# shenwei356/wfa

Hardware: AMD Instinct MI355X
Metric: aligned pairs/sec (and Gcells/s) on 1e6 synthetic 1 kbp pairs @5% error (higher is better)
Workload: dtype u32; 1 GPU; 1000000 x 1000 bp pairs/GPU @5% error, global gap-affine 4/6/2, wf-adaptive 10/50/1, seed 3; config=c3, pairs_per_gpu=1000000, length=1000, parallelism=pair-sharded x1, ranks_seen_by_collective=1, backend=none (1 GPU), collective_forced=False, status_ok=1000000, setup_steps=0, gather=none (1 GPU), gather_bytes_per_rank_step=0, packed_pairs=1000000, retried_pairs=831

## Files before the change

### wfa_amd/csrc/wfa_blk.hpp

```cpp
#pragma once
#include "wfa_device.hpp"
#include "wfa_packed.hpp"
#include <type_traits>

namespace wfa {

#ifndef WFA_BLK_TILED
#define WFA_BLK_TILED 1
#endif

template <int G>
struct BlkOps;

template <>
struct BlkOps<16> {
    static WFA_DEV uint32_t dn1(uint32_t x, int) { return (uint32_t)__builtin_amdgcn_update_dpp(0, (int)x, 0x111, 0xf, 0xf, true); }
    static WFA_DEV uint32_t up1(uint32_t x, int) { return (uint32_t)__builtin_amdgcn_update_dpp(0, (int)x, 0x101, 0xf, 0xf, true); }
#ifndef WFA_BLK_SHIFT_LANES
#define WFA_BLK_SHIFT_LANES 1
#endif
    static constexpr int SHIFT_D = 4 * WFA_BLK_SHIFT_LANES;
    static WFA_DEV uint32_t shr(uint32_t x, int) { return (uint32_t)__builtin_amdgcn_update_dpp(0, (int)x, 0x110 + WFA_BLK_SHIFT_LANES, 0xf, 0xf, true); }
    static WFA_DEV uint32_t shl(uint32_t x, int) { return (uint32_t)__builtin_amdgcn_update_dpp(0, (int)x, 0x100 + WFA_BLK_SHIFT_LANES, 0xf, 0xf, true); }
};

// ... 1045 lines not shown
        for (int i = 0; i < 8; i++) atomicAdd(acc + 8 + i, evt[i]);
    }
#endif
    if constexpr (STREAM) {
        stream_backtrace(P);
    }
    if constexpr (G == 64 && PP == 1 && !LONG) {
        if (P.fuse_bt) {
            if constexpr (LDSA) {
                __builtin_amdgcn_fence(__ATOMIC_ACQ_REL, "workgroup");
                if (lds[P.lds_arena_off - 4] != ST_OK) __threadfence();
                backtrace_wave_one<true>(P, blockIdx.x, lds + P.lds_arena_off);
            } else {
                __threadfence();
            }
            if constexpr (LDSA) {
            } else
                for (uint32_t idx = blockIdx.x; idx < P.chunk_n; idx += gridDim.x) backtrace_wave_one(P, idx, lds);
            if (lane == 0 && gridDim.x == 1u) *P.queue_head = 0u, *P.redo_count = 0u, *P.ops_cursor = 0ull;
        }
    }
}

WFA_DEV uint32_t prepack_dword(uint32_t w, bool &bad) {
    const uint32_t x = (w >> 1) & 0x03030303u;
    bad |= __builtin_amdgcn_perm(0u, 0x47544341u, x) != w;
    const uint32_t y = x | (x >> 6);
    return (y & 0xFu) | ((y >> 12) & 0xF0u);
}
WFA_DEV void prepack_fetch(const uint8_t *blob, uint64_t off, uint32_t len, uint32_t jw, uint32_t (&d)[5], uint32_t &sh, uint32_t &nb) {
    const uint32_t nw = (len + 15u) >> 4;
    sh = 0u, nb = 0u;
#pragma unroll
    for (int i = 0; i < 5; i++) d[i] = 0u;
    if (jw >= nw) return;
    const uintptr_t a  = (uintptr_t)(blob + off) + 16ull * jw;
    const uint32_t *p  = (const uint32_t *)(a & ~(uintptr_t)3);
    sh = (uint32_t)(a & 3) * 8u;
    nb = (len - 16u * jw) < 16u ? (len - 16u * jw) : 16u;
    const uint32_t  nd = ((uint32_t)(a & 3) + nb + 3u) >> 2;
    if ((a & 15) == 0 && nb == 16u) {
        const uint4 v = *reinterpret_cast<const uint4 *>(a);
        d[0] = v.x, d[1] = v.y, d[2] = v.z, d[3] = v.w, d[4] = 0u;
    } else {
#pragma unroll
        for (int i = 0; i < 5; i++) d[i] = ((uint32_t)i < nd) ? p[i] : 0u;
    }
}
WFA_DEV uint32_t prepack_finish(const uint32_t (&d)[5], uint32_t sh, uint32_t nb, bool &bad) {
    if (nb == 0u) return 0u;
    uint32_t word = 0u;
#pragma unroll
    for (int i = 0; i < 4; i++) {
        uint32_t w = __funnelshift_r(d[i], d[i + 1], sh);
        if (nb < 16u) {
            const uint32_t mb = nb > 4u * i ? (nb - 4u * i < 4u ? nb - 4u * i : 4u) : 0u;
            const uint32_t km = mb >= 4u ? 0xFFFFFFFFu : ((1u << (8u * mb)) - 1u);
            w = (w & km) | (0x41414141u & ~km);
        }
        word |= prepack_dword(w, bad) << (8 * i);
    }
    return word;
}
WFA_DEV uint32_t prepack_word(const uint8_t *blob, uint64_t off, uint32_t len, uint32_t jw, bool &bad) {
    uint32_t d[5], sh, nb;
    prepack_fetch(blob, off, len, jw, d, sh, nb);
    return prepack_finish(d, sh, nb, bad);
}

constexpr int PREPACK_PAIRS = 4;
#ifndef WFA_NO_AUX_KERNELS
__global__ __launch_bounds__(256) void wfa_prepack_kernel(const KParams P, uint32_t *out, uint32_t SW, uint32_t PW, uint32_t ppw) {
    const uint32_t lane = threadIdx.x & 63u;
    const uint32_t wv   = blockIdx.x * 4u + (threadIdx.x >> 6);
    const uint32_t LP = 2u * SW <= 32u ? 32u : 64u, side = lane / LP, v0 = lane % LP, n_side = 64u / LP;
    struct Hd { uint32_t nq, mt; uint64_t qo, to; };
    const auto load_hd = [&](uint32_t k) -> Hd {
        const uint32_t wi = wv * ppw + k + side;
        Hd h = {0u, 0u, 0ull, 0ull};
        if (k < ppw && wi < P.chunk_n) {
            const uint32_t pr = P.work ? P.work[wi] : P.chunk_first + wi;
            h.nq = P.q_len[pr], h.mt = P.t_len[pr], h.qo = P.q_off[pr], h.to = P.t_off[pr];
        }
        return h;
    };
    Hd nxt = load_hd(0);
    for (uint32_t k = 0; k < ppw; k += n_side) {
        const uint32_t wi = wv * ppw + k + side;
        if (wv * ppw + k >= P.chunk_n) return;
        const bool     have = wi < P.chunk_n;
        const Hd       cur  = nxt;
        nxt                 = load_hd(k + n_side);
// ... 32 lines not shown
```

### wfa_amd/csrc/wfa_ctx.hpp

```cpp
#pragma once
#include "../../include/wfa_hip.h"
#include "wfa_common.hpp"

#include <algorithm>
#include <atomic>
#include <chrono>
#include <cmath>
#include <cstdio>
#include <cstdlib>
#include <cstring>
#include <deque>
#include <functional>
#include <malloc.h>
#include <mutex>
#include <new>
#include <numeric>
#include <string>
#include <thread>
#include <vector>
#include <fcntl.h>
#include <optional>
#include <sys/file.h>
#include <unistd.h>

// ... 111 lines not shown
    int64_t       opt_arena_poison         = 0;
    int64_t       opt_pilot                = 1;
    int64_t       opt_tail_overlap         = 1;
    int64_t       opt_overlap              = 0;
    int64_t       opt_fail_pass            = 0;
    int64_t       opt_prepack              = 0;
    int64_t       opt_narrow_long          = 0;
    DevBuf        score_out;
    DevBuf        wide_ckpt;
    DevBuf        mx_seq, mx_words;
    DevBuf        mx_out;
    uint2        *mx_pin       = nullptr;
    size_t        mx_pin_bytes = 0;
    hipEvent_t    mx_ev[4]     = {};
    int64_t       opt_matrix_tile_cells    = 0;
    int64_t       opt_wide                 = 1;
    int64_t       opt_wide_max_len         = 2047;
    int           opt_wide_waves           = 0;
    bool          opt_wide_exact           = false;
    int64_t       opt_wide_min_pairs       = 64;
    int64_t       opt_duo                  = 1;
    int64_t       opt_duo_min_pairs        = 200000;
    bool          opt_duo_pk               = true;
    int64_t       opt_duo_short            = 0;
    int64_t       opt_duo_short_min_pairs  = 50000;
    bool          ctrl_clean               = false;
    hipStream_t   ctrl_clean_stream        = nullptr;
    hipEvent_t    ctrl_clean_ev            = nullptr;
    bool          redo_was_empty           = false;
    int64_t       opt_compact_call_bases   = 50000000;
    int64_t       opt_lane                 = 1;
    int64_t       opt_lane_pack            = 1;
    int64_t       opt_lane_min_pairs       = 32768;
    int64_t       opt_long                 = 1;
    int64_t       opt_long_min_len         = 4000;
    int64_t       opt_long_window_words    = 240;
    int64_t       opt_long_first           = 0;
    int64_t       opt_long_wave_bt         = 1;
    int64_t       opt_census               = 0;
    int64_t       opt_learn                = 1;
    uint64_t      learn_key                = 0;
    int           learn_level              = 0;
    uint32_t      learn_calls              = 0;
    uint64_t      rows_key                 = 0;
    uint32_t      rows_scale               = 1;
    uint64_t      band_key                 = 0;
// ... 59 lines not shown
```

### wfa_amd/csrc/wfa_duo.hip

```cpp
#define WFA_NO_AUX_KERNELS 1
#include "wfa_duo.hpp"
#include "wfa_fwd.hpp"

namespace wfa {

namespace {
template <int DX, int DOE>
hipError_t go_duo(const KParams &P, uint32_t grid, size_t lds_bytes, hipStream_t st, bool census, bool pk) {
    if (pk && census)
        hipLaunchKernelGGL((wfa_duo_kernel<true, DX, DOE>), dim3(grid), dim3(64), lds_bytes, st, P);
    else if (pk)
        hipLaunchKernelGGL((wfa_duo_kernel<false, DX, DOE>), dim3(grid), dim3(64), lds_bytes, st, P);
    else if (census)
        hipLaunchKernelGGL((wfa_duo32_kernel<true, DX, DOE>), dim3(grid), dim3(64), lds_bytes, st, P);
    else
        hipLaunchKernelGGL((wfa_duo32_kernel<false, DX, DOE>), dim3(grid), dim3(64), lds_bytes, st, P);
    return hipGetLastError();
}
}

hipError_t wfa_launch_duo(int shape, const KParams &P, uint32_t grid, size_t lds_bytes, hipStream_t st, bool census, bool pk) {
    switch (shape) {
    case 0: return go_duo<2, 4>(P, grid, lds_bytes, st, census, pk);
    case 1: return go_duo<1, 3>(P, grid, lds_bytes, st, census, pk);
    case 2: return go_duo<1, 2>(P, grid, lds_bytes, st, census, pk);
    case 3: return go_duo<2, 3>(P, grid, lds_bytes, st, census, pk);
    case 4: return go_duo<2, 2>(P, grid, lds_bytes, st, census, pk);
    case 5: return go_duo<3, 3>(P, grid, lds_bytes, st, census, pk);
    }
    return hipErrorInvalidValue;
}

}
```

### wfa_amd/csrc/wfa_duo.hpp

```cpp
#pragma once
#include "wfa_blk.hpp"
#include "wfa_duo_cfg.hpp"
#include "wfa_pk16.hpp"

namespace wfa {

struct DuoRed {
#define WFA_DUO_3(opa, opb, opc)                                                                                    \
    unsigned long long sv;                                                                                          \
    asm volatile("s_nop 1\n\t" opa " %0, %0, %0 " WFA_DPP_CTL_XOR1 "\n\t" opb " %1, %1, %1 " WFA_DPP_CTL_XOR1 "\n\t" opc \
        " %2, %2, %2 " WFA_DPP_CTL_XOR1 "\n\t" opa " %0, %0, %0 " WFA_DPP_CTL_XOR2 "\n\t" opb " %1, %1, %1 "        \
        WFA_DPP_CTL_XOR2 "\n\t" opc " %2, %2, %2 " WFA_DPP_CTL_XOR2 "\n\t" opa " %0, %0, %0 " WFA_DPP_CTL_HMIR "\n\t" \
        opb " %1, %1, %1 " WFA_DPP_CTL_HMIR "\n\t" opc " %2, %2, %2 " WFA_DPP_CTL_HMIR "\n\t"                         \
        "s_and_saveexec_b64 %3, %4\n\t" opa " %0, %0, %0 " WFA_DPP_CTL_MIR "\n\t" opb " %1, %1, %1 " WFA_DPP_CTL_MIR    \
        "\n\t" opc " %2, %2, %2 " WFA_DPP_CTL_MIR "\n\ts_mov_b64 exec, %3"                                            \
        : "+v"(a), "+v"(b), "+v"(c), "=&s"(sv)                                                                      \
        : "s"(wm)                                                                                                   \
        : "scc");
#define WFA_DUO_2(opa, opb)                                                                                         \
    unsigned long long sv;                                                                                          \
    asm volatile("s_nop 1\n\t" opa " %0, %0, %0 " WFA_DPP_CTL_XOR1 "\n\t" opb " %1, %1, %1 " WFA_DPP_CTL_XOR1 "\n\ts_nop 0\n\t" \
        opa " %0, %0, %0 " WFA_DPP_CTL_XOR2 "\n\t" opb " %1, %1, %1 " WFA_DPP_CTL_XOR2 "\n\ts_nop 0\n\t" opa        \
        " %0, %0, %0 " WFA_DPP_CTL_HMIR "\n\t" opb " %1, %1, %1 " WFA_DPP_CTL_HMIR "\n\t"                            \
        "s_and_saveexec_b64 %2, %3\n\t" opa " %0, %0, %0 " WFA_DPP_CTL_MIR "\n\t" opb " %1, %1, %1 " WFA_DPP_CTL_MIR    \
// ... 5 lines not shown
    unsigned long long sv;                                                                                          \
    asm volatile("s_nop 1\n\t" opa " %0, %0, %0 " WFA_DPP_CTL_XOR1 "\n\ts_nop 1\n\t" opa " %0, %0, %0 " WFA_DPP_CTL_XOR2 \
        "\n\ts_nop 1\n\t" opa " %0, %0, %0 " WFA_DPP_CTL_HMIR "\n\t"                                                \
        "s_and_saveexec_b64 %1, %2\n\ts_nop 0\n\t" opa " %0, %0, %0 " WFA_DPP_CTL_MIR "\n\ts_mov_b64 exec, %1"       \
        : "+v"(a), "=&s"(sv)                                                                                        \
        : "s"(wm)                                                                                                   \
        : "scc");
    static WFA_DEV void min_max_min(int &a, int &b, int &c, unsigned long long wm) { WFA_DUO_3("v_min_i32_dpp", "v_max_i32_dpp", "v_min_i32_dpp") }
    static WFA_DEV void min_max(int &a, int &b, unsigned long long wm) { WFA_DUO_2("v_min_i32_dpp", "v_max_i32_dpp") }
    static WFA_DEV void max_add(int &a, int &b, unsigned long long wm) { WFA_DUO_2("v_max_i32_dpp", "v_add_u32_dpp") }
    static WFA_DEV int  max1(int a, unsigned long long wm) {
        WFA_DUO_1("v_max_i32_dpp")
        return a;
    }
    static WFA_DEV int or1(int a, unsigned long long wm) {
        WFA_DUO_1("v_or_b32_dpp")
        return a;
    }
#undef WFA_DUO_3
#undef WFA_DUO_2
#undef WFA_DUO_1
};

template <bool CENSUS, int DX, int DOE, bool PK>
__device__ __attribute__((always_inline)) inline void duo_run(const KParams &P) {
    constexpr int PP = 4;
    static_assert(DX >= 1 && DOE >= 1 && DX <= 4 && DOE <= 4, "ring depths of one to four score steps");
    constexpr int R  = DX > DOE ? DX : DOE;
    constexpr int RW = PK ? 2 : PP;
    extern __shared__ __attribute__((aligned(16))) uint32_t lds[];
    const int  lane = threadIdx.x, l7 = lane & 7, l15 = lane & 15;
    const bool hi_half = (lane & 8) != 0;

    const uint32_t  SW = P.lds_seq_words, PW = P.prepack_words;
    const uint32_t  FP = duo_fetch_pairs(PW), NBUF = duo_bufs(PW);
    uint32_t *const park0 = lds + NBUF * PW;
    const uint64_t  cap      = P.arena_words;
    const int       mdd      = (int)P.max_dist_diff;
    const int       minwf    = (int)P.min_wf_len;
    const bool      adaptive = P.adaptive != 0;
    const uint32_t  seed_si  = P.dx;
    uint32_t        pk_one   = 0x00010001u;
    if constexpr (PK) asm volatile("" : "+s"(pk_one));
    const int       rows_cap = (int)(cap / 32);

    int       st = 0;
    bool      wide = false;
    uint32_t  pidx = 0, si = 0, cells = 0, sbuf = 0;
    int       n = 0, m = 0, kb = 0;
    bool      slow = false, first_eq = false;
    int             j = l7, k0 = 0;
    uint32_t        mdn = 0u, mup = 0u;
    const uint32_t *lq = lds + 4, *lt = lds + 4;
    uint32_t       *rowp = nullptr;

    uint32_t M[R][RW], I[RW], D[RW];
    int      rlo[R], rhi[R];
    int      lim[PP], lmx[PP];
#pragma unroll
    for (int d = 0; d < R; d++) {
        rlo[d] = BK_BIG, rhi[d] = -BK_BIG;
#pragma unroll
        for (int p = 0; p < RW; p++) M[d][p] = 0u;
    }
#pragma unroll
    for (int p = 0; p < RW; p++) I[p] = D[p] = 0u;
#pragma unroll
    for (int p = 0; p < PP; p++) lim[p] = 0, lmx[p] = 0;

    uint32_t buf_free  = (1u << NBUF) - 1u;
    uint32_t park_used = 0u;
    constexpr uint32_t PF_TOK = 1u, PF_LD = 2u, PF_STAGED = 4u, PF_DRY = 8u;
    uint32_t pf = 0u;
    uint32_t pf_tok = 0u, pf_ld_idx = 0u, pf_idx = 0u, pf_buf = 0u;
    uint32_t st_mask = 0u;
    uint4    pf_w = make_uint4(0u, 0u, 0u, 0u);

#ifdef WFA_STAMPS
    unsigned long long stamp_acc[8] = {0, 0, 0, 0, 0, 0, 0, 0}, stamp_prev;
    unsigned long long evt[8] = {0, 0, 0, 0, 0, 0, 0, 0};
    asm volatile("s_memtime %0\n\ts_waitcnt lgkmcnt(0)" : "=s"(stamp_prev)::"memory");
#endif
    const auto pair_of = [&](uint32_t idx) { return P.work ? P.work[idx] : P.chunk_first + idx; };
    const auto dn1 = [&](uint32_t x) { return (uint32_t)__builtin_amdgcn_update_dpp(0, (int)x, 0x111, 0xf, 0xf, true) & mdn; };
    const auto up1 = [&](uint32_t x) { return (uint32_t)__builtin_amdgcn_update_dpp(0, (int)x, 0x101, 0xf, 0xf, true) & mup; };
    const auto other_half = [&](int x) { return __builtin_amdgcn_update_dpp(0, x, 0x128, 0xf, 0xf, true); };
    const auto set_derived = [&]() {
        j   = wide ? l15 : l7;
        mdn = j == 0 ? 0u : ~0u;
        mup = j == (wide ? 15 : 7) ? 0u : ~0u;
        k0  = kb + PP * j;
#pragma unroll
        for (int p = 0; p < PP; p++) lim[p] = imax2(1, imin2(n + k0 + p, m)), lmx[p] = imax2(n + k0 + p, m);
        lq   = lds + sbuf * PW + 4u;
        lt   = lq + SW;
        if constexpr (DUO_ARENA_FMT == 10u)
            rowp = P.arena + (uint64_t)pidx * cap + (((uint32_t)k0 & 56u) >> 3) * (uint32_t)(rows_cap * 4) + (((uint32_t)k0 >> 2) & 1u) * 16u;
        else if constexpr (DUO_ARENA_FMT == 9u)
            rowp = P.arena + (uint64_t)pidx * cap + (((uint32_t)k0 & 60u) >> 2) * (uint32_t)(rows_cap * 2) + si * 2u;
        else
            rowp = P.arena + (uint64_t)pidx * cap + (uint64_t)(si >> 3) * 256u + (si & 7u) * 2u;
    };
    const auto clear_rings = [&]() {
#pragma unroll
        for (int d = 0; d < R; d++) {
            rlo[d] = BK_BIG, rhi[d] = -BK_BIG;
#pragma unroll
            for (int p = 0; p < RW; p++) M[d][p] = 0u;
        }
#pragma unroll
        for (int p = 0; p < RW; p++) I[p] = D[p] = 0u;
    };
    const auto or_halves = [&](uint32_t v) {
        uint32_t r = 0u;
#pragma unroll
        for (int o = 0; o < 8; o++) r |= (uint32_t)__builtin_amdgcn_readlane((int)v, 8 * o);
        return r;
    };

    const auto refill = [&](auto ph_c) __attribute__((always_inline)) -> bool {
        constexpr int ph  = decltype(ph_c)::value;
        constexpr int NEW = (ph + R - 1) % R;
        pf        = (uint32_t)__builtin_amdgcn_readfirstlane((int)pf);
        park_used = (uint32_t)__builtin_amdgcn_readfirstlane((int)park_used);
        buf_free  = (uint32_t)__builtin_amdgcn_readfirstlane((int)buf_free);
        st_mask   = (uint32_t)__builtin_amdgcn_readfirstlane((int)st_mask);
        if ((pf & (PF_LD | PF_STAGED)) == PF_LD) {
            const uint32_t cnt = umin2(FP, P.chunk_n - pf_ld_idx);
            st_mask = 0u;
            {
                uint32_t f = buf_free;
                for (uint32_t c = 0; c < cnt; c++) st_mask |= f & (0u - f), f &= f - 1u;
            }
            buf_free &= ~st_mask;
            const uint32_t w0 = (uint32_t)lane * 4u, slot = w0 / PW;
            if (slot < cnt) {
                uint32_t f = st_mask;
                for (uint32_t c = 0; c < slot; c++) f &= f - 1u;
                const uint32_t b = (uint32_t)__builtin_ctz(f);
                *reinterpret_cast<uint4 *>(lds + b * PW + (w0 - slot * PW)) = pf_w;
            }
            pf_idx = pf_ld_idx, pf = (pf | PF_STAGED) & ~PF_LD;
        }
        if ((pf & (PF_TOK | PF_LD)) == PF_TOK) {
            pf_ld_idx = (uint32_t)__builtin_amdgcn_readfirstlane((int)pf_tok);
            const bool have = pf_ld_idx < P.chunk_n;
            if (have) {
                const uint32_t *const slot = P.prepack + (uint64_t)pf_ld_idx * PW;
                const uint32_t cnt = umin2(FP, P.chunk_n - pf_ld_idx);
                if ((uint32_t)lane * 4u < cnt * PW) pf_w = *reinterpret_cast<const uint4 *>(slot + lane * 4);
            }
            pf = (pf & ~PF_TOK) | (have ? PF_LD : PF_DRY);
        }
        if ((pf & (PF_TOK | PF_DRY)) == 0u) {
            if (lane == 0) pf_tok = atomicAdd(P.queue_head, FP);
            pf |= PF_TOK;
        }
        unsigned long long m_free;
        WFA_STAMP(0);
        for (;;) {
        const bool run   = st == 1;
        const int  Wc    = wide ? 64 : 32;
        const bool touch = run && rhi[NEW] >= rlo[NEW] && (rlo[NEW] <= kb || rhi[NEW] >= kb + Wc - 1);
        bool       narrowable = false;
        if constexpr (ph == 0) {
            int ulo = rlo[0], uhi = rhi[0];
#pragma unroll
            for (int d = 1; d < R; d++) ulo = imin2(ulo, rlo[d]), uhi = imax2(uhi, rhi[d]);
            narrowable    = run && wide && uhi - ulo + 1 <= DUO_NARROW_AT;
        }
        const unsigned long long m_ev = __ballot(touch || narrowable);
        m_free = __ballot(st == 0);
        if (__builtin_expect(!(m_ev != 0ull || (m_free != 0ull && (park_used != 0u || (pf & PF_STAGED) != 0u))), 1)) break;
        WFA_EVT(1, 1);
        {
// ... 189 lines not shown
                    }
                    buf_free |= 1u << pf_buf;
                    continue;
                }
                WFA_EVT(5, 1);
                if (mine) {
                    pidx = this_idx, sbuf = pf_buf;
                    n = (int)nq, m = (int)mt;
                    const int Ak = m - n;
                    si = 0, cells = 0, slow = false;
                    kb = -16 + PP * imax2(-3, imin2(3, Ak / (2 * PP)));
                    first_eq = ((hb[4] ^ hb[4 + SW]) & 3u) == 0u;
                    clear_rings();
                    st = 1, wide = false;
                }
                m_free &= ~(0xFFull << (8 * oct));
            }
            set_derived();
            __builtin_amdgcn_fence(__ATOMIC_RELEASE, "wavefront");
            __builtin_amdgcn_fence(__ATOMIC_ACQUIRE, "wavefront");
        }
        }
        WFA_STAMP(1);
        return m_free == ~0ull && park_used == 0u && (pf & (PF_DRY | PF_LD | PF_STAGED)) == PF_DRY;
    };

    const auto step = [&](auto ph_c) __attribute__((always_inline)) {
        constexpr int ph = decltype(ph_c)::value;
        const bool run = (st == 1);
        const unsigned long long wm = __ballot(wide);
        WFA_EVT(0, 1), WFA_EVT(6, __builtin_popcountll(__ballot(run)) / 8);

        uint32_t(&Mo)[RW] = M[(ph + R - DOE) % R];
        uint32_t(&Mx)[RW] = M[(ph + R - DX) % R];
        uint32_t(&Mn)[RW] = M[ph];

        uint32_t nM[PP], nI[RW], nD[RW], wd[RW], cc[PP];
        const uint32_t a_edge = dn1(Mo[RW - 1]), b_edge = dn1(I[RW - 1]);
        const uint32_t c_edge = up1(Mo[0]), d_edge = up1(D[0]);
        const bool     slow_any = __ballot(run && slow) != 0ull;
        const auto next_slow = [&](const uint32_t(&Mo4)[PP], const uint32_t(&I4)[PP], const uint32_t(&D4)[PP], const uint32_t(&Mx4)[PP],
                                   uint32_t ae, uint32_t be, uint32_t ce, uint32_t de, uint32_t(&nI4)[PP], uint32_t(&nD4)[PP],
                                   uint32_t(&wd4)[PP]) __attribute__((always_inline)) {
#pragma unroll
            for (int p = 0; p < PP; p++) {
                const int      k  = k0 + p;
                const uint32_t a0 = p ? Mo4[p - 1] : ae, b0 = p ? I4[p - 1] : be;
// ... 289 lines not shown
            if (refill(std::integral_constant<int, 2 % R>{})) break;
            step(std::integral_constant<int, 2 % R>{});
        }
        if constexpr (R > 3) {
            if (refill(std::integral_constant<int, 3 % R>{})) break;
            step(std::integral_constant<int, 3 % R>{});
        }
    }
#ifdef WFA_STAMPS
    if (lane == 0 && P.debug_info) {
        unsigned long long *acc = reinterpret_cast<unsigned long long *>(P.debug_info);
        for (int i = 0; i < 8; i++) atomicAdd(acc + i, stamp_acc[i]);
        for (int i = 0; i < 8; i++) atomicAdd(acc + 8 + i, evt[i]);
    }
#endif
}

#ifndef WFA_DUO_VGPRS
#define WFA_DUO_VGPRS 64
#endif
static_assert(16u * (256u - 4u) / 2u < 2048u, "wfa_duo_kernel's packed rings need offsets under 4 096");
template <bool CENSUS, int DX = 2, int DOE = 4>
__global__ __launch_bounds__(64, WFA_DUO_WAVES) __attribute__((amdgpu_num_vgpr(WFA_DUO_VGPRS))) void wfa_duo_kernel(const KParams P) {
    duo_run<CENSUS, DX, DOE, true>(P);
}
template <bool CENSUS, int DX = 2, int DOE = 4>
__global__ __launch_bounds__(64, WFA_DUO_WAVES) __attribute__((amdgpu_num_vgpr(WFA_DUO_VGPRS))) void wfa_duo32_kernel(const KParams P) {
    duo_run<CENSUS, DX, DOE, false>(P);
}

}
```

### wfa_amd/csrc/wfa_host.hip

```cpp
#include <map>
#include "wfa_ctx.hpp"
#include "wfa_generic.hpp"
#include "wfa_packed.hpp"
#include "wfa_reg.hpp"
#include "wfa_blk.hpp"
#include "wfa_duo_cfg.hpp"
#include "wfa_lane.hpp"
#include "wfa_team.hpp"
#include "wfa_teamc.hpp"
#include "wfa_fwd.hpp"
#include "wfa_long.hpp"
#include "wfa_wide.hpp"

using namespace wfa;
static_assert(TEAM_SOLO_MAX == 4096, "wfa_ctx.hpp: default of opt_team_solo_max");

namespace wfa {
hipError_t wfa_launch_fwd(int shape, int kind, uint32_t flags, const KParams &P, uint32_t grid, size_t lds_bytes, hipStream_t st) {
    switch (shape) {
    case 0: return wfa_launch_fwd_s24(kind, flags, P, grid, lds_bytes, st);
    case 1: return wfa_launch_fwd_s13(kind, flags, P, grid, lds_bytes, st);
    case 2: return wfa_launch_fwd_s12(kind, flags, P, grid, lds_bytes, st);
    case 3: return wfa_launch_fwd_s23(kind, flags, P, grid, lds_bytes, st);
    case 4: return wfa_launch_fwd_s22(kind, flags, P, grid, lds_bytes, st);
// ... 382 lines not shown
        ctx->opt_pair_lds = value, ctx->one_lds_skip = 0;
    else if (k == "long_wave_bt")
        ctx->opt_long_wave_bt = value;
    else if (k == "long_min_len")
        ctx->opt_long_min_len = value;
    else if (k == "long_window_words")
        ctx->opt_long_window_words = (value >= 64 && value <= 4096 && value % 4 == 0) ? value : 240;
    else if (k == "wide")
        ctx->opt_wide = value;
    else if (k == "wide_min_pairs")
        ctx->opt_wide_min_pairs = value;
    else if (k == "matrix_tile_cells")
        ctx->opt_matrix_tile_cells = value > 0 ? value : 0;
    else if (k == "wide_max_len")
        ctx->opt_wide_max_len = value;
    else if (k == "wide_exact")
        ctx->opt_wide_exact = value != 0;
    else if (k == "wide_waves")
        ctx->opt_wide_waves = (value == 1 || value == 4) ? (int)value : 0;
    else if (k == "duo")
        ctx->opt_duo = value;
    else if (k == "duo_pk")
        ctx->opt_duo_pk = value != 0;
    else if (k == "duo_min_pairs")
        ctx->opt_duo_min_pairs = value;
    else if (k == "compact_call_bases")
        ctx->opt_compact_call_bases = value;
    else if (k == "lane")
        ctx->opt_lane = value;
    else if (k == "lane_pack")
        ctx->opt_lane_pack = value;
    else if (k == "lane_min_pairs")
        ctx->opt_lane_min_pairs = value;
    else if (k == "duo_short")
        ctx->opt_duo_short = value;
    else if (k == "duo_short_min_pairs")
        ctx->opt_duo_short_min_pairs = value;
    else if (k == "blk_mid")
        ctx->opt_blk_mid = value;
    else if (k == "pair_fast")
        ctx->opt_pair_fast = value;
    else if (k == "arena_budget_pct")
        ctx->opt_arena_budget_pct = value;
    else if (k == "autopack")
        ctx->opt_autopack = value;
    else if (k == "learn")
// ... 267 lines not shown
        HIP_TRY(hipMemsetAsync(stampbuf.p, 0, 128, st));
        P.debug_info = static_cast<uint32_t *>(stampbuf.p);
#endif
        uint64_t rkey = 0;
        {
            uint32_t lb = 0;
            while ((2u << lb) <= max_len) lb++;
            rkey = 1ull | ((uint64_t)lb << 1) | ((uint64_t)P.adaptive << 9) | ((uint64_t)(P.x & 0xFFF) << 12) | ((uint64_t)(P.oe & 0xFFF) << 24) |
                   ((uint64_t)(P.e & 0xFFF) << 36) | ((uint64_t)(P.max_dist_diff & 0xFFFF) << 48);
        }
        uint64_t arena_mult = (ctx->rows_key == rkey && ctx->opt_packed_arena_bytes <= 0) ? ctx->rows_scale : 1;
        auto forward_pass = [&](int kind, const std::vector<uint32_t> *list, uint64_t first_pair, uint64_t count,
                                std::vector<uint64_t> &redo_out, bool detach_bt) -> int {
            const uint32_t seq_words = fp_seq_words;
            const uint64_t words_dir = fp_words_dir;
            const bool second = ctx->bt_pending || (list && ctx->arena.bytes <= ctx->total_mem / 10);
            DevBuf &arena_buf = second ? ctx->arena2 : ctx->arena;
            DevBuf &meta_buf  = second ? ctx->meta2 : ctx->meta;
            const bool     blk_batch    = (kind == 3 || kind == 6) && seq_words <= 16 && ctx->opt_blk_batch != 0;
            if (kind == 6 && !blk_batch && ctx->opt_narrow_long == 0) return WFAHIP_ERR_INTERNAL;
            if (ctx->opt_fail_pass == kind) return WFAHIP_ERR_OOM;
            const uint32_t duo_sw       = (seq_words + 1u) & ~1u, duo_pw = 4u + 2u * duo_sw;
            if (kind == 8 && (duo_pw > 256u || blk_batch)) return WFAHIP_ERR_INTERNAL;
            if (kind == 10 && (seq_words > (uint32_t)LN_SEQ_WORDS || list)) return WFAHIP_ERR_INTERNAL;
            const uint32_t lane_sw      = (seq_words + 1u) & ~1u;
            const bool     is_long      = kind >= 11 && kind <= 15;
            const uint32_t long_sw      = (seq_words + 3u) & ~3u, long_cw = (uint32_t)ctx->opt_long_window_words;
            if (is_long && !can_long) return WFAHIP_ERR_INTERNAL;
            if (is_long && (uint64_t)seq_words * 16u < (uint64_t)max_len && !list) return WFAHIP_ERR_INTERNAL;
            const int      bkind        = (kind == 11 || kind == 14) ? 3 : (kind == 12 || kind == 15) ? 9 : kind == 13 ? 5 : kind;
            const size_t   lds_bytes    = is_long ? (size_t)(kind == 11 ? 4 : kind == 12 ? 2 : 1) * 2 * long_cw * 4
                                          : kind == 10 ? (size_t)64 * lane_stride_words(lane_sw) * 4
                                          : kind == 8 ? (size_t)duo_lds_words(duo_pw) * 4
                                          : kind == 9 ? (size_t)seq_words * 2 * 4 * 2 + 16
                                          : blk_batch ? (size_t)(kind == 6 ? 8 : 4) * BLK_BATCH * (2 * seq_words + 8) * 4 + 16
                                          : kind == 6 ? (size_t)seq_words * 2 * 4 * 8 + 16
                                          : kind == 5 ? (size_t)seq_words * 2 * 4 + 16
                                                      : (kind >= 3 ? lds_d : (kind == 2 ? lds_c : lds_b));
            const uint32_t pairs_wave   = kind >= 13 ? 1 : kind == 10 ? 64 : bkind == 5 ? 1 : bkind == 9 ? 2 : (kind == 4 || kind == 6 || kind == 8 ? 8 : (kind >= 2 ? 4 : 2));
            const uint64_t words        = bkind == 5   ? std::max<uint64_t>((words_dir * 16 * arena_mult + 511) & ~511ull, 8192)
                                          : bkind == 9 ? std::max<uint64_t>((words_dir * 4 * arena_mult + 511) & ~511ull, 4096)
                                          : kind == 8 ? std::max<uint64_t>((words_dir * arena_mult + 511) & ~511ull, 1024)
                                          : kind == 10 ? std::max<uint64_t>((words_dir * arena_mult + 511) & ~511ull, 1024)
                                          : kind >= 3 ? std::max<uint64_t>((words_dir * 2 * arena_mult + 511) & ~511ull, 2048)
                                                      : words_dir;
            P.arena_words = words, P.compact_fmt = kind == 10 ? 8u : kind == 8 ? DUO_ARENA_FMT : kind == 6 ? 5u : bkind == 5 ? 4u : bkind == 9 ? 6u : (kind >= 3 ? (WFA_BLK_TILED ? 3u : 1u) : 0u);
// ... 49 lines not shown
                hipEvent_t evBa = detach_bt ? ctx->evBtA : ctx->evpool[4 * c + 2];
                hipEvent_t evBb = detach_bt ? ctx->evBtB : ctx->evpool[4 * c + 3];
                const uint32_t buf = (uint32_t)(c % n_buf);
                P.arena       = static_cast<uint32_t *>(arena_buf.p) + (uint64_t)buf * chunk * words;
                P.pair_meta   = static_cast<uint4 *>(meta_buf.p) + (uint64_t)buf * chunk;
                P.chunk_first = (uint32_t)(first_pair + c0), P.chunk_n = (uint32_t)cn;
                P.work        = list ? static_cast<const uint32_t *>(ctx->work.p) + c0 : nullptr;
                if (!list && c == 0 && first_pair == 0)
                    ctx->dbg_arena = P.arena, ctx->dbg_meta = P.pair_meta, ctx->dbg_words = words, ctx->dbg_first = first_pair,
                    ctx->dbg_n = cn, ctx->dbg_fmt = P.compact_fmt, ctx->dbg_g = P.g;
                uint32_t grid = (uint32_t)std::min<uint64_t>((uint64_t)ctx->num_cus * waves_per_cu,
                                                            (cn + pairs_wave - 1) / pairs_wave);
                const uint32_t n_bt = stream_bt ? (uint32_t)std::min<int64_t>(ctx->opt_bt_stream, grid / 4) : 0u;
                if (stream_bt) {
                    if (grid < (uint32_t)ctx->num_cus * waves_per_cu) grid = std::min<uint32_t>(grid + n_bt, (uint32_t)ctx->num_cus * waves_per_cu);
                    P.n_stream_wgs = n_bt;
                    P.stream_wait  = (uint32_t)std::min<int64_t>(std::max<int64_t>(ctx->opt_bt_stream_wait_us, 0) * 100, 0x7FFFFFFF);
                    HIP_TRY(hipMemsetAsync(ctx->doneq.p, 0, 256 + 16 * cn, st));
                    HIP_TRY(hipMemsetAsync(P.pair_meta, 0xFF, 16 * cn, st));
                }
                P.prepack = nullptr, P.prepack_words = 0;
                P.lds_seq_words = is_long ? long_sw : kind == 10 ? lane_sw : kind == 8 ? duo_sw : seq_words;
                if (kind == 10) P.sub_lds_words = lane_stride_words(lane_sw);
                if ((kind == 3 && !blk_batch && !list && ctx->opt_prepack != 0) || kind == 8 || (kind == 10 && ctx->opt_lane_pack == 0) || is_long) {
                    const uint32_t pw = 4u + 2u * P.lds_seq_words;
                    if ((rc2 = ensure(ctx, ctx->prepack, (size_t)chunk * pw * 4))) return rc2;
                    if (ctx->pk_words)
                        hipLaunchKernelGGL(wfa_prepack_words_kernel, dim3((uint32_t)((cn + 3) / 4)), dim3(256), 0, st, P, ctx->pk_words,
                                           static_cast<uint32_t *>(ctx->prepack.p), P.lds_seq_words, pw);
                    else {
                        const uint32_t ppw = (cn <= (uint64_t)ctx->num_cus * 64 && 2u * P.lds_seq_words > 32u) ? 1u : (uint32_t)PREPACK_PAIRS;
                        hipLaunchKernelGGL(wfa_prepack_kernel, dim3((uint32_t)((cn + 4 * ppw - 1) / (4 * ppw))), dim3(256), 0, st, P,
                                           static_cast<uint32_t *>(ctx->prepack.p), P.lds_seq_words, pw, ppw);
                    }
                    HIP_TRY(hipGetLastError());
                    P.prepack = static_cast<const uint32_t *>(ctx->prepack.p), P.prepack_words = pw;
                } else if (ctx->pk_words) {
                    hipLaunchKernelGGL(wfa_unpack_pairs_kernel, dim3((uint32_t)((cn + 3) / 4)), dim3(256), 0, st, P, ctx->pk_words,
                                       const_cast<uint8_t *>(P.blob));
                    HIP_TRY(hipGetLastError());
                }
                if (is_long) P.lds_seq_words = long_cw;
                if (n_buf == 2 && c >= 2) HIP_TRY(hipStreamWaitEvent(st, ctx->evpool[4 * (c - 2) + 3], 0));
                if (c > 0) HIP_TRY(hipMemsetAsync(d_ctrl, 0, 4, st));
                if (ctx->opt_arena_poison) HIP_TRY(hipMemsetAsync(P.arena, 0xA5, (size_t)(words * 4ull * cn), st));
                HIP_TRY(hipEventRecord(evFa, st));
                if (kind == 8) {
// ... 703 lines not shown
```

Before: 62.56 million pairs/s.

## Fuse sequence prepacking into duo kernel's prefetch pipeline, skipping prepack pass

The duo alignment kernel can now read pair headers and raw ASCII sequence bytes straight from the blob inside its refill state machine. It converts them to 2-bit packed words across several rounds and writes them into LDS buffers, replacing the separate prepack kernel launch and its global staging buffer. This removes a full pass that writes and re-reads packed sequences in global memory, plus one kernel launch. The cost is extra packing work and global load latency interleaved with alignment steps, a more complex state machine, and more register pressure in the hot kernel. It only applies when one pair is fetched at a time and no work list or pk_words path is in use.

```diff
diff --git a/wfa_amd/csrc/wfa_blk.hpp b/wfa_amd/csrc/wfa_blk.hpp
--- a/wfa_amd/csrc/wfa_blk.hpp
+++ b/wfa_amd/csrc/wfa_blk.hpp
@@ -1,6 +1,7 @@
 #pragma once
 #include "wfa_device.hpp"
 #include "wfa_packed.hpp"
+#include "wfa_prepack.hpp"
 #include <type_traits>
 
 namespace wfa {
@@ -1092,52 +1093,6 @@
     }
 }
 
-WFA_DEV uint32_t prepack_dword(uint32_t w, bool &bad) {
-    const uint32_t x = (w >> 1) & 0x03030303u;
-    bad |= __builtin_amdgcn_perm(0u, 0x47544341u, x) != w;
-    const uint32_t y = x | (x >> 6);
-    return (y & 0xFu) | ((y >> 12) & 0xF0u);
-}
-WFA_DEV void prepack_fetch(const uint8_t *blob, uint64_t off, uint32_t len, uint32_t jw, uint32_t (&d)[5], uint32_t &sh, uint32_t &nb) {
-    const uint32_t nw = (len + 15u) >> 4;
-    sh = 0u, nb = 0u;
-#pragma unroll
-    for (int i = 0; i < 5; i++) d[i] = 0u;
-    if (jw >= nw) return;
-    const uintptr_t a  = (uintptr_t)(blob + off) + 16ull * jw;
-    const uint32_t *p  = (const uint32_t *)(a & ~(uintptr_t)3);
-    sh = (uint32_t)(a & 3) * 8u;
-    nb = (len - 16u * jw) < 16u ? (len - 16u * jw) : 16u;
-    const uint32_t  nd = ((uint32_t)(a & 3) + nb + 3u) >> 2;
-    if ((a & 15) == 0 && nb == 16u) {
-        const uint4 v = *reinterpret_cast<const uint4 *>(a);
-        d[0] = v.x, d[1] = v.y, d[2] = v.z, d[3] = v.w, d[4] = 0u;
-    } else {
-#pragma unroll
-        for (int i = 0; i < 5; i++) d[i] = ((uint32_t)i < nd) ? p[i] : 0u;
-    }
-}
-WFA_DEV uint32_t prepack_finish(const uint32_t (&d)[5], uint32_t sh, uint32_t nb, bool &bad) {
-    if (nb == 0u) return 0u;
-    uint32_t word = 0u;
-#pragma unroll
-    for (int i = 0; i < 4; i++) {
-        uint32_t w = __funnelshift_r(d[i], d[i + 1], sh);
-        if (nb < 16u) {
-            const uint32_t mb = nb > 4u * i ? (nb - 4u * i < 4u ? nb - 4u * i : 4u) : 0u;
-            const uint32_t km = mb >= 4u ? 0xFFFFFFFFu : ((1u << (8u * mb)) - 1u);
-            w = (w & km) | (0x41414141u & ~km);
-        }
-        word |= prepack_dword(w, bad) << (8 * i);
-    }
-    return word;
-}
-WFA_DEV uint32_t prepack_word(const uint8_t *blob, uint64_t off, uint32_t len, uint32_t jw, bool &bad) {
-    uint32_t d[5], sh, nb;
-    prepack_fetch(blob, off, len, jw, d, sh, nb);
-    return prepack_finish(d, sh, nb, bad);
-}
-
 constexpr int PREPACK_PAIRS = 4;
 #ifndef WFA_NO_AUX_KERNELS
 __global__ __launch_bounds__(256) void wfa_prepack_kernel(const KParams P, uint32_t *out, uint32_t SW, uint32_t PW, uint32_t ppw) {
diff --git a/wfa_amd/csrc/wfa_ctx.hpp b/wfa_amd/csrc/wfa_ctx.hpp
--- a/wfa_amd/csrc/wfa_ctx.hpp
+++ b/wfa_amd/csrc/wfa_ctx.hpp
@@ -157,6 +157,7 @@
     int64_t       opt_duo                  = 1;
     int64_t       opt_duo_min_pairs        = 200000;
     bool          opt_duo_pk               = true;
+    bool          opt_duo_selfpack         = true;
     int64_t       opt_duo_short            = 0;
     int64_t       opt_duo_short_min_pairs  = 50000;
     bool          ctrl_clean               = false;
diff --git a/wfa_amd/csrc/wfa_duo.hip b/wfa_amd/csrc/wfa_duo.hip
--- a/wfa_amd/csrc/wfa_duo.hip
+++ b/wfa_amd/csrc/wfa_duo.hip
@@ -7,10 +7,16 @@
 namespace {
 template <int DX, int DOE>
 hipError_t go_duo(const KParams &P, uint32_t grid, size_t lds_bytes, hipStream_t st, bool census, bool pk) {
-    if (pk && census)
+    if (!pk && !P.prepack) return hipErrorInvalidValue;
+    if (!P.prepack && (P.work || duo_fetch_pairs(P.prepack_words) != 1u)) return hipErrorInvalidValue;
+    if (pk && !P.prepack && census)
         hipLaunchKernelGGL((wfa_duo_kernel<true, DX, DOE>), dim3(grid), dim3(64), lds_bytes, st, P);
+    else if (pk && !P.prepack)
+        hipLaunchKernelGGL((wfa_duo_kernel<false, DX, DOE>), dim3(grid), dim3(64), lds_bytes, st, P);
+    else if (pk && census)
+        hipLaunchKernelGGL((wfa_duo_slot_kernel<true, DX, DOE>), dim3(grid), dim3(64), lds_bytes, st, P);
     else if (pk)
-        hipLaunchKernelGGL((wfa_duo_kernel<false, DX, DOE>), dim3(grid), dim3(64), lds_bytes, st, P);
+        hipLaunchKernelGGL((wfa_duo_slot_kernel<false, DX, DOE>), dim3(grid), dim3(64), lds_bytes, st, P);
     else if (census)
         hipLaunchKernelGGL((wfa_duo32_kernel<true, DX, DOE>), dim3(grid), dim3(64), lds_bytes, st, P);
     else
diff --git a/wfa_amd/csrc/wfa_duo.hpp b/wfa_amd/csrc/wfa_duo.hpp
--- a/wfa_amd/csrc/wfa_duo.hpp
+++ b/wfa_amd/csrc/wfa_duo.hpp
@@ -51,7 +51,7 @@
 #undef WFA_DUO_1
 };
 
-template <bool CENSUS, int DX, int DOE, bool PK>
+template <bool CENSUS, int DX, int DOE, bool PK, bool SELF>
 __device__ __attribute__((always_inline)) inline void duo_run(const KParams &P) {
     constexpr int PP = 4;
     static_assert(DX >= 1 && DOE >= 1 && DX <= 4 && DOE <= 4, "ring depths of one to four score steps");
@@ -62,7 +62,7 @@
     const bool hi_half = (lane & 8) != 0;
 
     const uint32_t  SW = P.lds_seq_words, PW = P.prepack_words;
-    const uint32_t  FP = duo_fetch_pairs(PW), NBUF = duo_bufs(PW);
+    const uint32_t  FP = SELF ? 1u : duo_fetch_pairs(PW), NBUF = duo_bufs(PW);
     uint32_t *const park0 = lds + NBUF * PW;
     const uint64_t  cap      = P.arena_words;
     const int       mdd      = (int)P.max_dist_diff;
@@ -99,11 +99,17 @@
 
     uint32_t buf_free  = (1u << NBUF) - 1u;
     uint32_t park_used = 0u;
-    constexpr uint32_t PF_TOK = 1u, PF_LD = 2u, PF_STAGED = 4u, PF_DRY = 8u;
-    uint32_t pf = 0u;
+    constexpr uint32_t PF_TOK = 1u, PF_LD = 2u, PF_STAGED = 4u, PF_DRY = 8u, PF_HDR = 16u, PF_BAD = 32u;
+    constexpr uint32_t PF_NOBUF = 0xFFu;
+    uint32_t pf = SELF ? PF_NOBUF << 16 : 0u;
     uint32_t pf_tok = 0u, pf_ld_idx = 0u, pf_idx = 0u, pf_buf = 0u;
     uint32_t st_mask = 0u;
     uint4    pf_w = make_uint4(0u, 0u, 0u, 0u);
+    uint32_t pf_hv = 0u, pf_hl = 0u, pf_x = 0u;
+    uint4    pf_v = make_uint4(0u, 0u, 0u, 0u);
+    const uint32_t *const pf_ha = lane == 0 ? P.q_len : lane == 1 ? P.t_len
+                                : lane < 4  ? reinterpret_cast<const uint32_t *>(P.q_off) + (lane - 2)
+                                            : reinterpret_cast<const uint32_t *>(P.t_off) + (lane - 4);
 
 #ifdef WFA_STAMPS
     unsigned long long stamp_acc[8] = {0, 0, 0, 0, 0, 0, 0, 0}, stamp_prev;
@@ -146,6 +152,44 @@
         for (int o = 0; o < 8; o++) r |= (uint32_t)__builtin_amdgcn_readlane((int)v, 8 * o);
         return r;
     };
+    const auto self_hdr    = [&](uint32_t hl, int i) { return (uint32_t)__builtin_amdgcn_readlane((int)hl, i); };
+    const auto self_status = [&](uint32_t n, uint32_t m) -> uint32_t {
+        if (n == 0u || m == 0u) return ST_EMPTY;
+        if (n > 0x1FFFFFFFu || m > 0x1FFFFFFFu) return ST_TOO_LONG;
+        if (((n > m ? n : m) + 15u) / 16u + 1u > SW) return ST_REDO_LDS;
+        return ST_PENDING;
+    };
+    const auto self_rounds = [&](uint32_t n, uint32_t m) -> uint32_t {
+        return self_status(n, m) == ST_PENDING ? (((n + 15u) >> 4) + ((m + 15u) >> 4) + 63u) >> 6 : 0u;
+    };
+    const auto self_word = [&](uint32_t hl, uint32_t r, uint64_t &off, uint32_t &len, uint32_t &jw, uint32_t &dst) {
+        const uint32_t n = self_hdr(hl, 0), m = self_hdr(hl, 1), nwq = (n + 15u) >> 4;
+        const uint64_t qo = (uint64_t)self_hdr(hl, 2) | ((uint64_t)self_hdr(hl, 3) << 32);
+        const uint64_t to = (uint64_t)self_hdr(hl, 4) | ((uint64_t)self_hdr(hl, 5) << 32);
+        const uint32_t w = 64u * r + (uint32_t)lane;
+        const bool     isq = w < nwq;
+        jw  = isq ? w : w - nwq;
+        len = isq ? n : m;
+        off = isq ? qo : to;
+        dst = 4u + (isq ? 0u : SW) + jw;
+    };
+    const auto self_fetch = [&](uint32_t hl, uint32_t r) {
+        uint64_t off;
+        uint32_t len, jw, dst, sh, nb;
+        self_word(hl, r, off, len, jw, dst);
+        prepack_load<false>(P.blob, off, len, jw, pf_v, pf_x, sh, nb);
+    };
+    const auto self_pack = [&](uint32_t hl, uint32_t r, uint32_t b) -> bool {
+        uint64_t off;
+        uint32_t len, jw, dst, sh, nb;
+        self_word(hl, r, off, len, jw, dst);
+        prepack_geom(P.blob, off, len, jw, sh, nb);
+        bool bad = false;
+        const uint32_t d[5] = {pf_v.x, pf_v.y, pf_v.z, pf_v.w, pf_x};
+        const uint32_t word = prepack_finish(d, sh, nb, bad);
+        if (nb != 0u) lds[b * PW + dst] = word;
+        return bad;
+    };
 
     const auto refill = [&](auto ph_c) __attribute__((always_inline)) -> bool {
         constexpr int ph  = decltype(ph_c)::value;
@@ -154,32 +198,73 @@
         park_used = (uint32_t)__builtin_amdgcn_readfirstlane((int)park_used);
         buf_free  = (uint32_t)__builtin_amdgcn_readfirstlane((int)buf_free);
         st_mask   = (uint32_t)__builtin_amdgcn_readfirstlane((int)st_mask);
-        if ((pf & (PF_LD | PF_STAGED)) == PF_LD) {
-            const uint32_t cnt = umin2(FP, P.chunk_n - pf_ld_idx);
-            st_mask = 0u;
-            {
-                uint32_t f = buf_free;
-                for (uint32_t c = 0; c < cnt; c++) st_mask |= f & (0u - f), f &= f - 1u;
-            }
-            buf_free &= ~st_mask;
-            const uint32_t w0 = (uint32_t)lane * 4u, slot = w0 / PW;
-            if (slot < cnt) {
-                uint32_t f = st_mask;
-                for (uint32_t c = 0; c < slot; c++) f &= f - 1u;
-                const uint32_t b = (uint32_t)__builtin_ctz(f);
-                *reinterpret_cast<uint4 *>(lds + b * PW + (w0 - slot * PW)) = pf_w;
-            }
-            pf_idx = pf_ld_idx, pf = (pf | PF_STAGED) & ~PF_LD;
-        }
-        if ((pf & (PF_TOK | PF_LD)) == PF_TOK) {
-            pf_ld_idx = (uint32_t)__builtin_amdgcn_readfirstlane((int)pf_tok);
-            const bool have = pf_ld_idx < P.chunk_n;
-            if (have) {
-                const uint32_t *const slot = P.prepack + (uint64_t)pf_ld_idx * PW;
+        if constexpr (SELF) {
+            if (pf & PF_LD) {
+                uint32_t r = (pf >> 8) & 0xFu, lb = (pf >> 16) & 0xFFu;
+                const uint32_t nr = (pf >> 12) & 0xFu;
+                if (r + 1u < nr || (pf & PF_STAGED) == 0u) {
+                    if (lb == PF_NOBUF && buf_free != 0u) lb = (uint32_t)__builtin_ctz(buf_free), buf_free &= buf_free - 1u;
+                    if (lb != PF_NOBUF) {
+                        if (r < nr) {
+                            if (__ballot(self_pack(pf_hl, r, lb)) != 0ull) pf |= PF_BAD;
+                            r += 1u;
+                            if (r < nr) self_fetch(pf_hl, r);
+                        }
+                        if (r >= nr) {
+                            const uint32_t n = self_hdr(pf_hl, 0), m = self_hdr(pf_hl, 1);
+                            const uint32_t status = (pf & PF_BAD) != 0u ? (uint32_t)ST_REDO_BYTES : self_status(n, m);
+                            if (lane == 0) *reinterpret_cast<uint4 *>(lds + lb * PW) = make_uint4(n, m, status, 0u);
+                            st_mask = 1u << lb, pf_idx = self_hdr(pf_hl, 6), lb = PF_NOBUF;
+                            pf = (pf | PF_STAGED) & ~(PF_LD | PF_BAD);
+                        }
+                    }
+                    pf = (pf & 0xF0FFu) | (r << 8) | (lb << 16);
+                }
+            }
+            if ((pf & (PF_HDR | PF_LD)) == PF_HDR) {
+                pf_hl = pf_hv;
+                const uint32_t nr = self_rounds(self_hdr(pf_hl, 0), self_hdr(pf_hl, 1));
+                if (nr != 0u) self_fetch(pf_hl, 0u);
+                pf = (pf & 0xFFu & ~(PF_HDR | PF_BAD)) | PF_LD | (nr << 12) | (PF_NOBUF << 16);
+            }
+            if ((pf & (PF_TOK | PF_HDR)) == PF_TOK) {
+                const uint32_t idx  = (uint32_t)__builtin_amdgcn_readfirstlane((int)pf_tok);
+                const bool     have = idx < P.chunk_n;
+                if (have) {
+                    asm volatile("v_writelane_b32 %0, %1, 6" : "+v"(pf_hv) : "s"(idx));
+                    const uint32_t pr = P.chunk_first + idx;
+                    if (lane < 6) pf_hv = pf_ha[(uint64_t)pr << (lane < 2 ? 0 : 1)];
+                }
+                pf = (pf & ~PF_TOK) | (have ? PF_HDR : PF_DRY);
+            }
+        } else {
+            if ((pf & (PF_LD | PF_STAGED)) == PF_LD) {
                 const uint32_t cnt = umin2(FP, P.chunk_n - pf_ld_idx);
-                if ((uint32_t)lane * 4u < cnt * PW) pf_w = *reinterpret_cast<const uint4 *>(slot + lane * 4);
-            }
-            pf = (pf & ~PF_TOK) | (have ? PF_LD : PF_DRY);
+                st_mask = 0u;
+                {
+                    uint32_t f = buf_free;
+                    for (uint32_t c = 0; c < cnt; c++) st_mask |= f & (0u - f), f &= f - 1u;
+                }
+                buf_free &= ~st_mask;
+                const uint32_t w0 = (uint32_t)lane * 4u, slot = w0 / PW;
+                if (slot < cnt) {
+                    uint32_t f = st_mask;
+                    for (uint32_t c = 0; c < slot; c++) f &= f - 1u;
+                    const uint32_t b = (uint32_t)__builtin_ctz(f);
+                    *reinterpret_cast<uint4 *>(lds + b * PW + (w0 - slot * PW)) = pf_w;
+                }
+                pf_idx = pf_ld_idx, pf = (pf | PF_STAGED) & ~PF_LD;
+            }
+            if ((pf & (PF_TOK | PF_LD)) == PF_TOK) {
+                pf_ld_idx = (uint32_t)__builtin_amdgcn_readfirstlane((int)pf_tok);
+                const bool have = pf_ld_idx < P.chunk_n;
+                if (have) {
+                    const uint32_t *const slot = P.prepack + (uint64_t)pf_ld_idx * PW;
+                    const uint32_t cnt = umin2(FP, P.chunk_n - pf_ld_idx);
+                    if ((uint32_t)lane * 4u < cnt * PW) pf_w = *reinterpret_cast<const uint4 *>(slot + lane * 4);
+                }
+                pf = (pf & ~PF_TOK) | (have ? PF_LD : PF_DRY);
+            }
         }
         if ((pf & (PF_TOK | PF_DRY)) == 0u) {
             if (lane == 0) pf_tok = atomicAdd(P.queue_head, FP);
@@ -415,7 +500,7 @@
         }
         }
         WFA_STAMP(1);
-        return m_free == ~0ull && park_used == 0u && (pf & (PF_DRY | PF_LD | PF_STAGED)) == PF_DRY;
+        return m_free == ~0ull && park_used == 0u && (pf & (PF_DRY | PF_HDR | PF_LD | PF_STAGED)) == PF_DRY;
     };
 
     const auto step = [&](auto ph_c) __attribute__((always_inline)) {
@@ -751,11 +836,15 @@
 static_assert(16u * (256u - 4u) / 2u < 2048u, "wfa_duo_kernel's packed rings need offsets under 4 096");
 template <bool CENSUS, int DX = 2, int DOE = 4>
 __global__ __launch_bounds__(64, WFA_DUO_WAVES) __attribute__((amdgpu_num_vgpr(WFA_DUO_VGPRS))) void wfa_duo_kernel(const KParams P) {
-    duo_run<CENSUS, DX, DOE, true>(P);
+    duo_run<CENSUS, DX, DOE, true, true>(P);
+}
+template <bool CENSUS, int DX = 2, int DOE = 4>
+__global__ __launch_bounds__(64, WFA_DUO_WAVES) __attribute__((amdgpu_num_vgpr(WFA_DUO_VGPRS))) void wfa_duo_slot_kernel(const KParams P) {
+    duo_run<CENSUS, DX, DOE, true, false>(P);
 }
 template <bool CENSUS, int DX = 2, int DOE = 4>
 __global__ __launch_bounds__(64, WFA_DUO_WAVES) __attribute__((amdgpu_num_vgpr(WFA_DUO_VGPRS))) void wfa_duo32_kernel(const KParams P) {
-    duo_run<CENSUS, DX, DOE, false>(P);
+    duo_run<CENSUS, DX, DOE, false, false>(P);
 }
 
 }
diff --git a/wfa_amd/csrc/wfa_host.hip b/wfa_amd/csrc/wfa_host.hip
--- a/wfa_amd/csrc/wfa_host.hip
+++ b/wfa_amd/csrc/wfa_host.hip
@@ -428,6 +428,8 @@
         ctx->opt_duo = value;
     else if (k == "duo_pk")
         ctx->opt_duo_pk = value != 0;
+    else if (k == "duo_selfpack")
+        ctx->opt_duo_selfpack = value != 0;
     else if (k == "duo_min_pairs")
         ctx->opt_duo_min_pairs = value;
     else if (k == "compact_call_bases")
@@ -741,6 +743,8 @@
             if (ctx->opt_fail_pass == kind) return WFAHIP_ERR_OOM;
             const uint32_t duo_sw       = (seq_words + 1u) & ~1u, duo_pw = 4u + 2u * duo_sw;
             if (kind == 8 && (duo_pw > 256u || blk_batch)) return WFAHIP_ERR_INTERNAL;
+            const bool     duo_self     = kind == 8 && !ctx->pk_words && !list && duo_fetch_pairs(duo_pw) == 1u && ctx->opt_duo_pk &&
+                                          ctx->opt_duo_selfpack;
             if (kind == 10 && (seq_words > (uint32_t)LN_SEQ_WORDS || list)) return WFAHIP_ERR_INTERNAL;
             const uint32_t lane_sw      = (seq_words + 1u) & ~1u;
             const bool     is_long      = kind >= 11 && kind <= 15;
@@ -836,7 +840,9 @@
                 P.prepack = nullptr, P.prepack_words = 0;
                 P.lds_seq_words = is_long ? long_sw : kind == 10 ? lane_sw : kind == 8 ? duo_sw : seq_words;
                 if (kind == 10) P.sub_lds_words = lane_stride_words(lane_sw);
-                if ((kind == 3 && !blk_batch && !list && ctx->opt_prepack != 0) || kind == 8 || (kind == 10 && ctx->opt_lane_pack == 0) || is_long) {
+                if (duo_self) {
+                    P.prepack_words = duo_pw;
+                } else if ((kind == 3 && !blk_batch && !list && ctx->opt_prepack != 0) || kind == 8 || (kind == 10 && ctx->opt_lane_pack == 0) || is_long) {
                     const uint32_t pw = 4u + 2u * P.lds_seq_words;
                     if ((rc2 = ensure(ctx, ctx->prepack, (size_t)chunk * pw * 4))) return rc2;
                     if (ctx->pk_words)
diff --git a/wfa_amd/csrc/wfa_prepack.hpp b/wfa_amd/csrc/wfa_prepack.hpp
--- /dev/null
+++ b/wfa_amd/csrc/wfa_prepack.hpp
@@ -0,0 +1,67 @@
+#pragma once
+#include "wfa_device.hpp"
+
+namespace wfa {
+
+WFA_DEV uint32_t prepack_dword(uint32_t w, bool &bad) {
+    const uint32_t x = (w >> 1) & 0x03030303u;
+    bad |= __builtin_amdgcn_perm(0u, 0x47544341u, x) != w;
+    const uint32_t y = x | (x >> 6);
+    return (y & 0xFu) | ((y >> 12) & 0xF0u);
+}
+template <bool X4 = true>
+WFA_DEV void prepack_load(const uint8_t *blob, uint64_t off, uint32_t len, uint32_t jw, uint4 &v, uint32_t &x, uint32_t &sh, uint32_t &nb) {
+    typedef const __attribute__((address_space(1))) uint32_t *gp32;
+    typedef uint32_t u32x4 __attribute__((ext_vector_type(4)));
+    typedef const __attribute__((address_space(1))) u32x4    *gp128;
+    const uint32_t nw = (len + 15u) >> 4;
+    sh = 0u, nb = 0u;
+    v = make_uint4(0u, 0u, 0u, 0u), x = 0u;
+    if (jw >= nw) return;
+    const uintptr_t a  = (uintptr_t)(blob + off) + 16ull * jw;
+    const gp32      p  = (gp32)(a & ~(uintptr_t)3);
+    sh = (uint32_t)(a & 3) * 8u;
+    nb = (len - 16u * jw) < 16u ? (len - 16u * jw) : 16u;
+    const uint32_t  nd = ((uint32_t)(a & 3) + nb + 3u) >> 2;
+    if (X4 && (a & 15) == 0 && nb == 16u) {
+        const u32x4 t = *(gp128)a;
+        v = make_uint4(t.x, t.y, t.z, t.w);
+    } else {
+        uint32_t d[5];
+#pragma unroll
+        for (int i = 0; i < 5; i++) d[i] = ((uint32_t)i < nd) ? p[i] : 0u;
+        v = make_uint4(d[0], d[1], d[2], d[3]), x = d[4];
+    }
+}
+WFA_DEV void prepack_fetch(const uint8_t *blob, uint64_t off, uint32_t len, uint32_t jw, uint32_t (&d)[5], uint32_t &sh, uint32_t &nb) {
+    uint4 v;
+    prepack_load(blob, off, len, jw, v, d[4], sh, nb);
+    d[0] = v.x, d[1] = v.y, d[2] = v.z, d[3] = v.w;
+}
+WFA_DEV uint32_t prepack_finish(const uint32_t (&d)[5], uint32_t sh, uint32_t nb, bool &bad) {
+    if (nb == 0u) return 0u;
+    uint32_t word = 0u;
+#pragma unroll
+    for (int i = 0; i < 4; i++) {
+        uint32_t w = __funnelshift_r(d[i], d[i + 1], sh);
+        if (nb < 16u) {
+            const uint32_t mb = nb > 4u * i ? (nb - 4u * i < 4u ? nb - 4u * i : 4u) : 0u;
+            const uint32_t km = mb >= 4u ? 0xFFFFFFFFu : ((1u << (8u * mb)) - 1u);
+            w = (w & km) | (0x41414141u & ~km);
+        }
+        word |= prepack_dword(w, bad) << (8 * i);
+    }
+    return word;
+}
+WFA_DEV uint32_t prepack_word(const uint8_t *blob, uint64_t off, uint32_t len, uint32_t jw, bool &bad) {
+    uint32_t d[5], sh, nb;
+    prepack_fetch(blob, off, len, jw, d, sh, nb);
+    return prepack_finish(d, sh, nb, bad);
+}
+WFA_DEV void prepack_geom(const uint8_t *blob, uint64_t off, uint32_t len, uint32_t jw, uint32_t &sh, uint32_t &nb) {
+    const uint32_t nw = (len + 15u) >> 4;
+    sh = (uint32_t)((uintptr_t)(blob + off) & 3) * 8u;
+    nb = jw >= nw ? 0u : ((len - 16u * jw) < 16u ? (len - 16u * jw) : 16u);
+}
+
+}
```

Result: no change. 63.02 million pairs/s, median of 6 (+0.7%).
